# 3decomp/poissbox

Hardware: AMD Instinct MI355X
Metric: CG iter/s and DoF-updates/s at 512^3; achieved HBM GB/s vs peak (higher is better)
Workload: dtype f64

## Files before the change

### poissbox_amd/csrc/pb_cg_device.hpp

```cpp
#pragma once

#include <type_traits>
#include <utility>
#include "pb_device.hpp"

namespace pb {

__device__ __forceinline__ bool finite(double v) { return v == v && v - v == 0.0; }
__device__ __forceinline__ double norm_from_sq(double zz) { return sqrt(zz < 0.0 ? 0.0 : zz); }
template <class S>
__device__ __forceinline__ void ablate_keep_going(S& st) {
#ifdef PB_ABLATE_NO_EXITS
  if (st.reason != PB_KSP_DIVERGED_ITS) st.reason = 0, st.done = 0;
#endif
}

static constexpr int kFoldMaxParts = 1024;
static constexpr int kMaxSums = 5;
__device__ __forceinline__ void wave_reduce_parts(const double* __restrict__ parts, int nparts,
                                                  int width, double* S) {
  const int lane = threadIdx.x & 63;
#pragma unroll
  for (int s = 0; s < kMaxSums; ++s) {
    double v = 0.0;
// ... 165 lines not shown
    } else if (skip && i + 1 >= st.max_it) {
      st.beta = zr;
      st.mu = mu;
      st.delta = S[4];
      st.it = i + 1;
      st.reason = PB_KSP_CONVERGED_ITS;
      st.done = 1;
    } else {
      st.beta = zr;
      st.mu = mu;
      st.delta = S[4];
      st.it = i + 1;
      if (!finite(zr)) {
        st.reason = PB_KSP_DIVERGED_NANORINF;
        st.done = 1;
      } else if (st.it >= st.max_it) {
        st.reason = PB_KSP_DIVERGED_ITS;
        st.done = 1;
      } else if (zr == 0.0) {
        st.its = st.it + 1;
        st.reason = PB_KSP_CONVERGED_ATOL;
        st.done = 1;
      } else if (zr * st.betaold < 0.0) {
        st.its = st.it + 1;
        st.reason = PB_KSP_DIVERGED_INDEFINITE_PC;
        st.done = 1;
      }
    }
  }
  ablate_keep_going(st);
  if (h_done) h_done[host_iter + 1] = st.done;
}

__device__ __forceinline__ void cg_sr_top(CgState& st) {
  if (st.done) return;
  const double dpi = st.it == 0 ? st.delta
                                : st.delta - st.beta * st.beta * st.dpi / (st.betaold * st.betaold);
  cg_stage1(st, dpi, false);
  if (!st.done) cg_pend(st);
}


__device__ __forceinline__ void cg_copy(CgState& d, const CgState& s) {
  d.beta = s.beta, d.betaold = s.betaold, d.dpi = s.dpi, d.dpiold = s.dpiold;
  d.alpha = s.alpha, d.alpha_prev = s.alpha_prev, d.mu = s.mu, d.dp = s.dp, d.ttol = s.ttol;
  d.rnorm0 = s.rnorm0, d.pa[0] = s.pa[0], d.pa[1] = s.pa[1], d.pa[2] = s.pa[2];
  d.rtol = s.rtol, d.atol = s.atol, d.dtol = s.dtol, d.dinv = s.dinv, d.ntot = s.ntot;
  d.it = s.it, d.its = s.its, d.max_it = s.max_it, d.nhist = s.nhist, d.pend_iter = s.pend_iter;
  d.pend_count = s.pend_count, d.nlog = s.nlog;
  d.reason = s.reason, d.done = s.done, d.pc = s.pc, d.nullspace = s.nullspace;
  d.defer_x = s.defer_x;
  d.bbp = s.bbp;
  d.delta = s.delta, d.sr = s.sr, d.norm = s.norm;
}
static_assert(sizeof(CgState) == 248, "cg_copy lists every CgState field");

__device__ __forceinline__ void fold_prologue(const Fold& f, CgState& st) {
  double S[kMaxSums];
  cg_copy(st, *f.in);
  if (f.stage != 4) wave_reduce_parts(f.parts, f.nparts, f.width, S);
  const bool lead = blockIdx.x == 0 && threadIdx.x == 0;
  if (f.stage == 1) {
    cg_stage1(st, S[0]);
  } else if (f.stage == 2) {
    cg_stage2(st, S, lead ? f.hist : nullptr, lead ? f.h_done : nullptr, f.host_iter);
  } else {
// ... 58 lines not shown
```

### poissbox_amd/csrc/pb_cg_passes.hip

```cpp
#include "pb_star7.hpp"

namespace pb {

struct CombineLoad {
  static constexpr int NR = 2;
  static constexpr bool GHOST_RAW = false;
  const double* __restrict__ r;
  const double* __restrict__ p;
  const CgState* st;
  double dinv, shift, bb;
  int after1 = 0;
  __device__ __forceinline__ void prepare() { prepare_from(*st); }
  template <class S>
  __device__ __forceinline__ void prepare_from(const S& s) {
    dinv = s.dinv;
    shift = -s.mu;
    bb = after1 ? s.bbp : (s.it == 0 ? 0.0 : s.beta / s.betaold);
  }
  __device__ __forceinline__ const double* src(int a) const { return a == 0 ? r : p; }
  __device__ __forceinline__ double f(double rv, double pv) const {
    double z = dinv * rv;
    z = z + shift;
    return z + bb * pv;
  }
// ... 499 lines not shown
                          double* p_new, const StencilPlanes& gp, const Fold& fold, int mode,
                          int part_off, int* nblocks, bool store) {
  ScopedTimer tm(g->ctx,
                 timer_name(mode, "cg_pass_a", "cg_pass_a_interior", "cg_pass_a_boundary"));
  const CombineLoad ld{r, p_old, nullptr, 0.0, 0.0, 0.0};
  Launch lc = Launch{nullptr, mode}.sums(part_off, nblocks);
  lc.fold = fold;
  if (!store) return launch_any(g, s, ld, gp, PassAT<false>{p_new}, lc);
  return launch_any(g, s, ld, gp, PassA{p_new}, lc);
}

int cg_reduce_allreduce(pb_ctx* ctx, int nparts, int width, bool b_region) {
  return cg_reduce_allreduce(ctx, ctx->d_partials + (b_region ? fold_parts_b_off(ctx) * 4 : 0),
                             nparts, width);
}

int cg_reduce_allreduce(pb_ctx* ctx, const double* parts, int nparts, int width) {
  hipLaunchKernelGGL(cg_finalize_kernel, dim3(1), dim3(256), 0, ctx->stream, parts, nparts, width,
                     ctx->d_scalars, 1, 0, (CgState*)nullptr, (double*)nullptr, (int*)nullptr,
                     (int64_t)0, RrParts{});
  PB_HIP(hipGetLastError());
  return allreduce_device(ctx, ctx->d_scalars, width);
}

int cg_stage2_from_sums(pb_ctx* ctx, int width, CgState* st, double* hist, int* h_done,
                        int64_t host_iter) {
  hipLaunchKernelGGL(cg_finalize_kernel, dim3(1), dim3(256), 0, ctx->stream,
                     (const double*)nullptr, 0, width, ctx->d_scalars, 2, 2, st, hist, h_done,
                     host_iter, RrParts{});
  PB_HIP(hipGetLastError());
  return PB_OK;
}

int cg_finalize_init(pb_ctx* ctx, int nparts, CgState* st, double* hist, int* h_done,
                     const RrParts& rr) {
  return cg_reduce_update(ctx, 0, nparts, 4, st, hist, h_done, -1, nullptr, rr);
}

int cg_finalize_pass_a(pb_ctx* ctx, int nparts, CgState* st) {
  return cg_reduce_update(ctx, 1, nparts, 1, st, nullptr, nullptr, 0);
}

int cg_finalize_stage2(pb_ctx* ctx, int nparts, CgState* st, double* hist, int* h_done,
                       int64_t host_iter, const RrParts& rr) {
  return cg_reduce_update(ctx, 2, nparts, 4, st, hist, h_done, host_iter, nullptr, rr);
}

template <int XU, bool PST>
static int pass_b_one(pb_grid* g, const Star& s, const double* p, const double* const* p_prev,
                      double* x, double* r, const StencilPlanes& gp, CgState* st, const Fold& f,
                      const PStore& ps, int* nparts, int part_off = 0) {
  const int* skip = f.stage ? nullptr : &st->done;
  const int off = f.stage ? (int)fold_parts_b_off(g->ctx) : part_off;
  Launch lc = Launch{skip}.sums(off, nparts);
  lc.rev = 1;
  lc.fold = f;
  PassB<XU, PST> ep{x, r, p_prev[0], XU == 3 ? p_prev[1] : nullptr, XU == 3 ? p_prev[2] : nullptr,
                    st, 0.0, 0.0, 0.0, 0.0, 0.0, 0.0};
  if constexpr (PST) {
    ep.r_out = ps.r_out;
    ep.p_out = const_cast<double*>(p);
    CombineLoad ld{ps.zsrc, p_prev[0], st, 0.0, 0.0, 0.0};
    ld.after1 = 1;
    return launch_any(g, s, ld, gp, ep, lc);
  } else {
    return launch_any(g, s, PlainLoad{p}, gp, ep, lc);
// ... 151 lines not shown
```

### poissbox_amd/csrc/pb_fft.hip

```cpp
#include <algorithm>
#include <cmath>
#include <vector>

#include "pb_internal.hpp"
#include "pb_device.hpp"

#pragma clang fp contract(fast)

namespace pb {

namespace {

struct DhtPass {
  const double* in;
  double* out;
  int64_t li, lo, es;
  int64_t lo_out;
  int esh_in, esh_out;
  int64_t ebs_in, ebs_out, es_out;
  int ninner, nouter, ntiles_inner;
  const double* w;
  const double* tab;
  int nx, ny, j0;
  double scale, thr;
  int remap;
  const double* sr;
  double* parts;
  const CgState* st;
  int nparts_out;
  int ncu;
  const double* ru_in;
  const double* ru_w;
  double* ru_out;
  const double* ru_p;
  double* ru_x;
  int ru_first;
  const CgState* ru_st;
  const double* in_alt = nullptr;
  double* out_alt = nullptr;
  int alt_blk = -1;
  int ablate;
};
#ifndef PB_FFT_ABLATE_TRAFFIC
#define PB_FFT_ABLATE_TRAFFIC 0
#endif

struct cplx {
  double re, im;
};
typedef double dv2 __attribute__((ext_vector_type(2)));
__device__ __forceinline__ cplx cmul(cplx a, cplx b) {
  return {a.re * b.re - a.im * b.im, a.re * b.im + a.im * b.re};
}
__device__ __forceinline__ cplx cadd(cplx a, cplx b) { return {a.re + b.re, a.im + b.im}; }
__device__ __forceinline__ cplx csub(cplx a, cplx b) { return {a.re - b.re, a.im - b.im}; }
__device__ __forceinline__ cplx cmi(cplx a) { return {a.im, -a.re}; }
__device__ __forceinline__ cplx cpi(cplx a) { return {-a.im, a.re}; }
__device__ __forceinline__ cplx cscale(cplx a, double s) { return {a.re * s, a.im * s}; }

__host__ __device__ constexpr int natural_radix_at(int n, int p) {
  int rest = n;
  for (int q = 0; q <= p; ++q) {
// ... 359 lines not shown
    const int f = fv + q * NS;
    if (NP % NS != 0 && f >= NP) {
      l = TL;
      e = 0;
    } else if (WAVE) {
      l = l0 + f / (N / 2);
      e = (f % (N / 2)) * 2;
    } else {
      l = (f % (TL / 2)) * 2;
      e = f / (TL / 2);
    }
  };
  constexpr bool PF = LAYOUT == 1 && N <= 512;
  dv2 pre[PF ? NR : 1];
  auto load_pair = [&](int64_t base, int nl, int q) -> dv2 {
    int l, e;
    coord(q, l, e);
    const bool ok = l < nl;
    const int lc = ok ? l : 0, ec = ok ? e : 0;
    if (PB_FFT_ABLATE_TRAFFIC) return dv2{0.0, 0.0};
    const double* src = p.in;
    if (LAYOUT == 0 && p.esh_in && (ec >> p.esh_in) == p.alt_blk) src = p.in_alt;
    return __builtin_nontemporal_load((const dv2*)(src + base + lc * p.li + eoff_in(ec)));
  };
  auto fetch = [&](int t) {
    int64_t outer, base;
    int inner0, nl;
    tile_of(t, outer, inner0, nl, base);
    if constexpr (PF) {
#pragma unroll
      for (int q = 0; q < NR; ++q) pre[q] = load_pair(base, nl, q);
    }
  };
  double acc[4] = {0.0, 0.0, 0.0, 0.0};
  const double mu = SUMS ? p.st->mu : 0.0;
  const int G = PF ? (int)gridDim.x : ntiles;
  int t = PF ? (int)blockIdx.x : xcd_block(p.remap);
  if (PF && t < ntiles) fetch(t);
  for (; t < ntiles; t += G) {
    int64_t outer, base;
    int inner0, nl;
    tile_of(t, outer, inner0, nl, base);

    if (WAVE)
      wave_sync_lds();
    else
      __syncthreads();
    auto put = [&](int l, int e, dv2 v) {
      if (LAYOUT == 0) {
        lds[l * LP + lpad(e)] = v.x;
        lds[(l + 1) * LP + lpad(e)] = v.y;
      } else {
        lds[l * LP + lpad(e)] = v.x;
        lds[l * LP + lpad(e + 1)] = v.y;
      }
    };
    if constexpr (PF) {
#pragma unroll
      for (int q = 0; q < NR; ++q) {
        int l, e;
        coord(q, l, e);
        if (l < nl) put(l, e, pre[q]);
      }
    } else {
      constexpr int QB = N <= 512 ? (NR < 8 ? NR : 8) : 4;
#pragma unroll
      for (int q0 = 0; q0 < NR; q0 += QB) {
        dv2 v[QB];
// ... 22 lines not shown
        fft_passes<N, 0, 1>(A, B, tw, lane);
        scale_combine2<N>(A, B, p, lane, outer, inner0 + l0);
        fft_passes<N, 0, 1>(A, B, tw, lane);
      } else {
        dht2<N>(A, B, tw, lane);
      }
    }
    if (WAVE)
      wave_sync_lds();
    else
      __syncthreads();
#pragma unroll
    for (int q = 0; q < NR; ++q) {
      int l, e;
      coord(q, l, e);
      if (l < nl) {
        dv2 v;
        if (LAYOUT == 0) {
          v.x = lds[l * LP + lpad(e)];
          v.y = lds[(l + 1) * LP + lpad(e)];
          if (MODE == 1) v.y = -v.y;
        } else {
          v.x = lds[l * LP + lpad(e)];
          v.y = lds[l * LP + lpad(e + 1)];
        }
        const int64_t a = base + outer * (p.lo_out - p.lo) + l * p.li + eoff_out(e);
        if (PB_FFT_ABLATE_TRAFFIC) {
          if (v.x == 12345.678) p.out[a] = v.y;
          continue;
        }
        double* dst = p.out;
        if (LAYOUT == 0 && p.esh_out && (e >> p.esh_out) == p.alt_blk) dst = p.out_alt;
        __builtin_nontemporal_store(v, (dv2*)(dst + a));
        if constexpr (SUMS) {
          const dv2 rv = __builtin_nontemporal_load((const dv2*)(p.sr + a));
          const double t0 = v.x - mu, t1 = v.y - mu;
          acc[0] += t0;
          acc[1] += t0 * t0;
          acc[2] += t0 * rv.x;
          acc[3] += rv.x;
          acc[0] += t1;
          acc[1] += t1 * t1;
          acc[2] += t1 * rv.y;
          acc[3] += rv.y;
        }
      }
    }
  }
  if constexpr (SUMS) {
    __syncthreads();
#pragma unroll
    for (int q = 0; q < 4; ++q) {
      double v = acc[q];
#pragma unroll
      for (int off = 32; off >= 1; off >>= 1) v += __shfl_xor(v, off, 64);
      if (lane == 0) lds[wave * 4 + q] = v;
    }
    __syncthreads();
    if (threadIdx.x < 4) {
      double v = lds[threadIdx.x];
      for (int w = 1; w < NT / 64; ++w) v += lds[w * 4 + threadIdx.x];
      p.parts[(int64_t)blockIdx.x * 4 + threadIdx.x] = v;
    }
  }
}

template <int N, bool SUMS, bool RUPD>
__global__ __launch_bounds__(512, N <= 512 ? 4 : 2) void dht_reg_x_kernel(DhtPass p,
                                                                          const int* skip) {
  static_assert(!(SUMS && RUPD), "sums on the last pass, the r update on the first");
  using RP = RegPlan<N>;
  static_assert(RP::OK, "register-edge plan");
  constexpr int R = RP::R, NB = RP::NB, T = RP::T;
  constexpr int TL = 16, LP = (lpad_max(N) + 1) | 1;
  constexpr bool TWL = N <= 512;
  if (skip && *skip) {
    if (RUPD && p.ru_first) {
      const int tile = blockIdx.x;
      const int64_t outer = tile / p.ntiles_inner;
      const int inner0 = (tile % p.ntiles_inner) * TL;
      const int nl = min(TL, p.ninner - inner0);
      for (int i = threadIdx.x; i < nl * N; i += 512)
        p.ru_x[outer * p.lo + (int64_t)(inner0 + i / N) * p.li + i % N] = 0.0;
    }
    return;
  }
  extern __shared__ __attribute__((aligned(16))) double lds[];
  const int lane = threadIdx.x & 63, wave = threadIdx.x >> 6;
  const double* tw = p.w;
  if constexpr (TWL) {
    double* twl = lds + TL * LP;
    for (int i = threadIdx.x; i < N; i += 512) {
      const dv2 c = *(const dv2*)(p.w + 2 * i);
      twl[2 * i] = c.x;
      twl[2 * i + 1] = c.y;
// ... 122 lines not shown
      PB_HIP(hipFuncSetAttribute((const void*)k, hipFuncAttributeMaxDynamicSharedMemorySize,
                                 (int)LDS));
    attr = true;
  }
  if (p.ru_st) {
    if (p.parts) return set_error(PB_ERR_STATE, "fft pc: r update and sums on one pass");
    kern = kern_r;
  }
  if (ntiles > INT32_MAX) return set_error(PB_ERR_UNSUPPORTED, "fft pc: too many tiles");
  int64_t nblocks = ntiles;
  if (p.parts) {
    static int occ = 0;
    if (!occ) {
      PB_HIP(hipOccupancyMaxActiveBlocksPerMultiprocessor(&occ, kern_s, 512, LDS));
      if (occ < 1) occ = 1;
    }
    nblocks = std::min<int64_t>(ntiles, (int64_t)occ * ctx->num_cus);
    if (nblocks * 4 > ctx->partials_cap)
      return set_error(PB_ERR_UNSUPPORTED, "fft pc: %lld blocks exceed the partials capacity",
                       (long long)nblocks);
    p.nparts_out = (int)nblocks;
    kern = kern_s;
  }
  hipLaunchKernelGGL(kern, dim3((unsigned)nblocks), dim3(512), LDS, ctx->stream, p, skip);
  PB_HIP(hipGetLastError());
  return PB_OK;
}

template <int N, int TL, int LAYOUT, int MODE>
int launch_dht_k(pb_ctx* ctx, DhtPass& p, const int* skip) {
  using T = DhtTile<N, TL>;
  p.ntiles_inner = (p.ninner + T::TL - 1) / T::TL;
  const int64_t ntiles = (int64_t)p.ntiles_inner * p.nouter;
  constexpr bool SUMS = LAYOUT == 1 && MODE == 0;
  auto kern = dht_lines_kernel<N, TL, LAYOUT, MODE, false>;
  auto kern_s = dht_lines_kernel<N, TL, LAYOUT, MODE, SUMS>;
  static int occ = 0;
  if (!occ) {
    PB_HIP(hipFuncSetAttribute((const void*)kern, hipFuncAttributeMaxDynamicSharedMemorySize,
                               (int)T::LDS));
    PB_HIP(hipFuncSetAttribute((const void*)kern_s, hipFuncAttributeMaxDynamicSharedMemorySize,
                               (int)T::LDS));
    PB_HIP(hipOccupancyMaxActiveBlocksPerMultiprocessor(&occ, kern_s, T::NT, T::LDS));
    if (occ < 1) occ = 1;
  }
  int64_t nblocks = (int64_t)occ * ctx->num_cus;
  const bool persist = N <= 512 && LAYOUT == 1;
  if (!persist || nblocks > ntiles) nblocks = ntiles;
  if (p.parts) {
    if (!SUMS) return set_error(PB_ERR_STATE, "fft pc: residual sums on the X pass only");
    if (nblocks * 4 > ctx->partials_cap)
      return set_error(PB_ERR_UNSUPPORTED, "fft pc: %lld blocks exceed the partials capacity",
                       (long long)nblocks);
    p.nparts_out = (int)nblocks;
    kern = kern_s;
  }
  hipLaunchKernelGGL(kern, dim3((unsigned)nblocks), dim3(T::NT), T::LDS, ctx->stream, p, skip);
  PB_HIP(hipGetLastError());
  return PB_OK;
}

template <int N, int LAYOUT, int MODE>
int launch_dht_n(pb_ctx* ctx, DhtPass& p, const int* skip) {
  if (p.ninner % 2)
    return set_error(PB_ERR_UNSUPPORTED, "fft pc: %d lines (even counts only)", p.ninner);
  if constexpr (RegPlan<N>::OK && LAYOUT == 1) return launch_dht_reg_x<N>(ctx, p, skip);
  if (p.ru_st) return set_error(PB_ERR_STATE, "fft pc: r update on the register-edge X pass only");
  return launch_dht_k<N, tile_lines<N>(), LAYOUT, MODE>(ctx, p, skip);
}

#define PB_FFT_LENGTHS(X) \
  X(32) X(64) X(128) X(256) X(512) X(1024) X(48) X(96) X(192) X(384) X(768) X(40) X(80) \
  X(160) X(320) X(640)

template <int LAYOUT, int MODE>
int launch_dht(pb_ctx* ctx, int64_t n, DhtPass& p, const int* skip) {
  switch (n) {
#define PB_FFT_CASE(L)                                                 \
  case L:                                                              \
    static_assert(plan_complete(L), "length without a Stockham plan"); \
    return launch_dht_n<L, LAYOUT, MODE>(ctx, p, skip);
    PB_FFT_LENGTHS(PB_FFT_CASE)
#undef PB_FFT_CASE
  }
// ... 99 lines not shown
  }
  pb_ctx* ctx = g->ctx;
  PB_HIP(hipMemcpyAsync(f->dev, host.data(), host.size() * sizeof(double), hipMemcpyHostToDevice,
                        ctx->stream));
  PB_SYNC(ctx, "fft pc tables");
  f->tw[0] = f->dev;
  f->tw[1] = f->dev + 2 * g->n[0];
  f->tw[2] = f->dev + 2 * (g->n[0] + g->n[1]);
  f->tab = f->dev + 2 * nsum;
  if (grid_split(g)) {
    const int64_t len = yslab_len(g) + yslab_aux_len(g);
    if (hipMalloc(&f->ybuf, (size_t)len * sizeof(double)) != hipSuccess) {
      (void)hipFree(f->dev);
      delete f;
      return set_error(PB_ERR_ALLOC, "fft pc y-slab buffer: out of device memory");
    }
  } else if (const int64_t pad = tune("fft_zpad", 32);
             pad > 0 && g->plane >= tune("fft_zpad_min_plane", 512 * 512)) {
    f->zplane = g->plane + pad;
    if (hipMalloc(&f->zbuf, (size_t)(f->zplane * g->nzl) * sizeof(double)) != hipSuccess) {
      (void)hipGetLastError();
      f->zbuf = nullptr;
      f->zplane = 0;
    }
  }
  *out = f;
  return PB_OK;
}

static int dht_axis(pb_ctx* ctx, const FftPc* f, const int64_t b[3], int axis, const double* in,
                    double* out, const int* skip, int j0 = 0, const double* sr = nullptr,
                    const CgState* st = nullptr, int* np = nullptr,
                    const RUpdate* ru = nullptr, int64_t pl_in = 0, int64_t pl_out = 0,
                    const YSlabPlan* blk = nullptr, int blk_dir = 0) {
  static const char* names[3] = {"pc_fft_x", "pc_fft_y", "pc_fft_z"};
  ScopedTimer tm(ctx, names[axis]);
  DhtPass p{};
  p.remap = 1;
  p.ablate = PB_ABLATE_FFT;
  p.ncu = ctx->num_cus;
  p.in = in;
  p.out = out;
  p.w = f->tw[axis];
  const int64_t nx = b[0], ny = b[1], nz = b[2];
  if (axis == 0) {
    p.li = nx;
    p.lo = nx * ny;
    p.lo_out = p.lo;
    p.es = 1;
    p.ninner = (int)ny;
    p.nouter = (int)nz;
    if (np) {
      p.sr = sr;
      p.st = st;
      p.parts = ctx->d_partials;
    }
    if (ru) {
      p.ru_in = ru->r_in;
      p.ru_w = ru->w;
      p.ru_out = ru->r_out;
      p.ru_p = ru->p;
      p.ru_x = ru->x;
      p.ru_first = ru->first;
      p.ru_st = ru->st;
    }
    PB_TRY((launch_dht<1, 0>(ctx, nx, p, skip)));
    if (np) *np = p.nparts_out;
// ... 9 lines not shown
    if (blk) {
      const int64_t nyl = blk->nyl[0];
      int sh = 0;
      while (((int64_t)1 << sh) < nyl) ++sh;
      if (blk_dir == 1) {
        p.lo_out = nyl * nx;
        p.esh_out = sh;
        p.ebs_out = nz * nyl * nx;
      } else {
        p.lo = nyl * nx;
        p.esh_in = sh;
        p.ebs_in = nz * nyl * nx;
      }
      if (blk->self_direct) {
        p.alt_blk = blk->me;
        p.out_alt = blk->alt_out;
        p.in_alt = blk->alt_out;
      }
    }
    return launch_dht<0, 0>(ctx, ny, p, skip);
  }
  p.li = 1;
  p.lo = nx;
  p.lo_out = nx;
  p.es = pl_in ? pl_in : nx * ny;
  p.ninner = (int)nx;
  p.nouter = (int)ny;
  p.tab = f->tab;
  p.nx = (int)f->g->n[0];
  p.ny = (int)f->g->n[1];
  p.j0 = j0;
  p.scale = 1.0 / ((double)f->g->n[0] * (double)f->g->n[1] * (double)f->g->n[2]);
  p.thr = f->thr;
  return launch_dht<0, 1>(ctx, nz, p, skip);
}

bool fftpc_fuses_r_update(const FftPc* f) {
  return (f->g->n[0] == 512 || f->g->n[0] == 1024) && f->g->n[1] % 2 == 0;
}

int fftpc_apply(FftPc* f, const double* r, double* z, const int* skip, const CgState* sums_st,
                int* nparts, const RUpdate* ru) {
  if (nparts) *nparts = 0;
  pb_grid* g = f->g;
  pb_ctx* ctx = g->ctx;
  if (ru && !fftpc_fuses_r_update(f))
    return set_error(PB_ERR_STATE, "fft pc: r update needs the register-edge X pass");
  ScopedTimer tm(ctx, "pc_fft");
  const int64_t b[3] = {g->n[0], g->n[1], g->nzl};
  PB_TRY(dht_axis(ctx, f, b, 0, r, z, skip, 0, nullptr, nullptr, nullptr, ru));
  if (f->zbuf) {
    PB_TRY(dht_axis(ctx, f, b, 1, z, f->zbuf, skip, 0, nullptr, nullptr, nullptr, nullptr, 0,
                    f->zplane));
    PB_TRY(dht_axis(ctx, f, b, 2, f->zbuf, f->zbuf, skip, 0, nullptr, nullptr, nullptr, nullptr,
                    f->zplane, f->zplane));
    PB_TRY(dht_axis(ctx, f, b, 1, f->zbuf, z, skip, 0, nullptr, nullptr, nullptr, nullptr,
                    f->zplane, 0));
  } else if (!grid_split(g)) {
    PB_TRY(dht_axis(ctx, f, b, 1, z, z, skip));
    PB_TRY(dht_axis(ctx, f, b, 2, z, z, skip));
    PB_TRY(dht_axis(ctx, f, b, 1, z, z, skip));
  } else {
    YSlabPlan yp;
    double* fy = f->ybuf;
    PB_TRY(yslab_begin(g, fy + yslab_len(g), &yp));
    const int64_t by[3] = {g->n[0], yp.ny_me, g->n[2]};
    if (yslab_blocked(yp)) {
      yp.alt_out = fy + yp.self_shift;
      PB_TRY(dht_axis(ctx, f, b, 1, z, yp.stage, skip, 0, nullptr, nullptr, nullptr, nullptr, 0,
                      0, &yp, 1));
      PB_TRY(alltoallv_device(ctx, yp.stage, yp.zc.data(), fy, yp.yc.data(), yp.self_direct));
      PB_TRY(dht_axis(ctx, f, by, 2, fy, fy, skip, (int)yp.j0[ctx->rank]));
      PB_TRY(alltoallv_device(ctx, fy, yp.yc.data(), yp.stage, yp.zc.data(), yp.self_direct));
      PB_TRY(dht_axis(ctx, f, b, 1, yp.stage, z, skip, 0, nullptr, nullptr, nullptr, nullptr, 0,
                      0, &yp, 2));
    } else {
      PB_TRY(dht_axis(ctx, f, b, 1, z, z, skip));
      PB_TRY(yslab_to(g, yp, z, fy));
      PB_TRY(dht_axis(ctx, f, by, 2, fy, fy, skip, (int)yp.j0[ctx->rank]));
      PB_TRY(yslab_from(g, yp, fy, z));
      PB_TRY(dht_axis(ctx, f, b, 1, z, z, skip));
    }
  }
  if (sums_st && nparts) return dht_axis(ctx, f, b, 0, z, z, skip, 0, r, sums_st, nparts);
  return dht_axis(ctx, f, b, 0, z, z, skip);
}

void fftpc_destroy(FftPc* f) {
  if (!f) return;
  (void)wait_stream(f->g->ctx, f->g->ctx->stream, "fftpc_destroy");
  if (f->dev) (void)hipFree(f->dev);
  if (f->ybuf) (void)hipFree(f->ybuf);
  if (f->zbuf) (void)hipFree(f->zbuf);
  delete f;
}

}
```

### poissbox_amd/csrc/pb_internal.hpp

```cpp
#pragma once

#include <hip/hip_runtime.h>
#include <rccl/rccl.h>
#include <rocprofiler-sdk-roctx/roctx.h>

#include <cstdint>
#include <cstdio>
#include <deque>
#include <map>
#include <string>
#include <functional>
#include <vector>

#include "poissbox_gpu.h"

namespace pb {

int set_error(int code, const char* fmt, ...);

#define PB_HIP(call)                                                                    \
  do {                                                                                  \
    hipError_t e_ = (call);                                                             \
    if (e_ != hipSuccess)                                                               \
      return ::pb::set_error(PB_ERR_HIP, "%s:%d %s: %s", __FILE__, __LINE__, #call,     \
// ... 446 lines not shown
                       const double* q, const double* b, double* y_out, double* r_out,
                       const StencilPlanes& gp, const CgState* st, double scale, bool sums,
                       int* nparts, int part_off = 0);
int launch_cheb_x(pb_grid* g, const double* y, const double* ym1, const double* q, double* y_out,
                  const CgState* st, double scale);
int launch_pre_scale_sum(pb_grid* g, const double* src, double* dst, double dinv, int* nparts);
int launch_pre_shift(pb_grid* g, double* x, double ntot);

struct Mg;
int mg_create(pb_grid* g, const double deltas[3], int pc_type, int levels_req, int coarse_its,
              double omega, Mg** out);
int mg_apply(Mg* mg, const double* r, double* z, const int* skip = nullptr,
             const CgState* sums_st = nullptr, int* nparts = nullptr);
int mg_levels(const Mg* mg);
struct MgSmoother {
  int ksp = 0, pc = 0, nu = 1;
  double rich_scale = 1.0, emin = 0.0, emax = 0.0;
};
int mg_set_smoother(Mg* mg, const MgSmoother& sm);
void mg_destroy(Mg* mg);
int mg_plan_levels(const int64_t n[3], int nranks, int levels_req);

struct FftPc;
int fftpc_create(pb_grid* g, const double deltas[3], int compact, FftPc** out);
struct RUpdate {
  const double* r_in;
  const double* w;
  double* r_out;
  const double* p;
  double* x;
  int first;
  const CgState* st;
};
int fftpc_apply(FftPc* f, const double* r, double* z, const int* skip = nullptr,
                const CgState* sums_st = nullptr, int* nparts = nullptr,
                const RUpdate* ru = nullptr);
bool fftpc_fuses_r_update(const FftPc* f);
void fftpc_destroy(FftPc* f);

int ctx_scratch(pb_ctx* ctx, size_t n, double** out);

int reduce_partials(pb_ctx* ctx, const double* parts, int nparts, int width, double* out);

}
```

### poissbox_amd/csrc/pb_ksp.hpp

```cpp
#pragma once
#include <vector>

#include "pb_internal.hpp"

namespace pb {
struct FgState;
struct PcgState;
}

struct pb_ksp {
  pb_op* A = nullptr;
  pb_op* P = nullptr;
  pb_ksp_opts opts;
  int norm_type = PB_KSP_NORM_DEFAULT;
  int norm() const {
    if (norm_type != PB_KSP_NORM_DEFAULT) return norm_type;
    if (opts.ksp_type == PB_KSP_FGMRES) return PB_KSP_NORM_UNPRECONDITIONED;
    return opts.ksp_type == PB_KSP_PREONLY ? PB_KSP_NORM_NONE : PB_KSP_NORM_PRECONDITIONED;
  }
  bool norm_none() const { return norm() == PB_KSP_NORM_NONE; }
  bool norm_unp() const { return norm() == PB_KSP_NORM_UNPRECONDITIONED; }
  int64_t solve_iters() const {
    return norm_none() ? opts.max_it : opts.max_it + 2 * (int64_t)opts.check_every;
  }
// ... 66 lines not shown
  pb_vec* x = nullptr;
  int64_t host_iter = 0;
  bool stopped = false;
  bool begun = false;
  int defer_x = 4;
  int pslots() const { return defer_x == 4 ? 4 : 2; }
  struct Sr {
    bool on = false;
    int nparts = 0;
  };
  Sr sr;
  struct Fischer {
    int maxl = 0, curl = 0;
    std::vector<double*> xt, bt;
    double* guess = nullptr;
    double* d_coef = nullptr;
  };
  Fischer* fg = nullptr;
};

#pragma GCC visibility push(hidden)
namespace pb {

inline bool fused_kind(int kind) { return kind == PB_OP_STAR7; }

int op_apply_raw(pb_op* op, const double* x, double* y);
struct OpApplySkip {
  pb_ctx* ctx;
  OpApplySkip(pb_ctx* c, const int* flag) : ctx(c) { ctx->op_skip = flag; }
  ~OpApplySkip() { ctx->op_skip = nullptr; }
};

int ensure_done_cap(pb_ksp* k, int64_t need);
int pc_apply_dev(pb_ksp* k, const double* r, double* z, const int* skip, int* np);

int check_cheb_pair(double emin, double emax, const char* what);
int check_cheb_opts(const pb_ksp_chebyshev_opts* o);
int check_mg_opts(const pb_pc_mg_opts* o);
int check_guess_opts(int model, int maxl);
int check_ref_norm_opts(const pb_ksp_opts* o);
int check_richardson_scale(double scale);
void mg_levels_bounds(const pb_pc_mg_opts* o, double* emin, double* emax);

int rich_begin(pb_ksp* k, const pb_vec* b, pb_vec* x);
int enqueue_rich_iteration(pb_ksp* k);
int rich_copy_back(pb_ksp* k, int64_t its);
int solve_preonly(pb_ksp* k, const pb_vec* b, pb_vec* x, pb_ksp_result* res);

int fgmres_create(pb_ksp* k);
int fgmres_begin(pb_ksp* k, const pb_vec* b, pb_vec* x);
int enqueue_fgmres_iteration(pb_ksp* k);
int fgmres_finish(pb_ksp* k);
void fgmres_destroy(pb_ksp* k);
int check_fgmres_opts(const pb_ksp_fgmres_opts* o);

constexpr int kFgMaxRestart = 64;
constexpr int kFgLd = kFgMaxRestart + 1;
struct FgState {
  double hh[kFgLd * kFgMaxRestart];
  double cs[kFgMaxRestart], sn[kFgMaxRestart];
  double g[kFgLd];
  double y[kFgMaxRestart];
  double dots[kFgLd], dots2[kFgLd];
  double nrm2;
  double wsum;
  double shift;
  double bsq;
// ... 61 lines not shown
```

### poissbox_amd/csrc/pb_runtime.cpp

```cpp
#include <time.h>

#include <algorithm>
#include <atomic>
#include <chrono>
#include <cstdarg>
#include <cstdlib>
#include <cstring>
#include <condition_variable>
#include <memory>
#include <mutex>
#include <string>
#include <thread>
#include <unordered_map>

#include "pb_internal.hpp"

namespace pb {

hipError_t field_alloc(void** p, size_t bytes) { return hipMalloc(p, bytes); }

void field_free(void* p) {
  if (p) (void)hipFree(p);
}

namespace {
const char* const kTuneNames[] = {
    "a2a_copy_self", "cg_defer_x", "engine_kc_skew", "cg_fold", "cg_fuse", "cg_sr_fused", "cheb_fused", "comm_mark_every",
    "comm_stall_test_ms", "compact_lines", "fft_rupd", "fgmres_fused", "pipecg_fused", "fft_zpad", "fft_zpad_min_plane",
    "force_comm", "ksp_lazy0", "mg_agglomerate", "mg_engine_min_plane", "mg_poly_fused", "mg_restrict_z_min_cols",
    "mg_split_fused", "mg_sweep2", "mg_tail_max", "mg_u4_split", "pcr_lines", "rich_fused", "sor_omega_any", "sr_ddiff",
    "stencil_kc", "stencil_kc_skew", "stencil_nt", "stencil_tall", "stencil_wgcu", "x_dot_cu"};
constexpr int kNumTune = (int)(sizeof(kTuneNames) / sizeof(kTuneNames[0]));
std::atomic<int> g_tune_val[kNumTune];
std::atomic<int> g_tune_set[kNumTune];
std::atomic<int> g_tune_nset{0};
int tune_index(const char* name) {
  for (int i = 0; i < kNumTune; ++i)
    if (strcmp(kTuneNames[i], name) == 0) return i;
  return -1;
}
}

int tune(const char* name, int dflt) {
  if (g_tune_nset.load(std::memory_order_acquire) == 0) return dflt;
  const int i = tune_index(name);
  if (i < 0 || !g_tune_set[i].load(std::memory_order_acquire)) return dflt;
  return g_tune_val[i].load(std::memory_order_relaxed);
}

bool tune_is_set(const char* name) {
  const int i = tune_index(name);
  return i >= 0 && g_tune_set[i].load(std::memory_order_acquire) != 0;
}

static thread_local char g_err[1024] = "";

int set_error(int code, const char* fmt, ...) {
  va_list ap;
  va_start(ap, fmt);
  vsnprintf(g_err, sizeof(g_err), fmt, ap);
  va_end(ap);
// ... 1027 lines not shown
```

### poissbox_amd/csrc/pb_solver.cpp

```cpp
#include <cmath>
#include <cstdio>
#include <cstring>
#include <string>
#include <vector>

#include "pb_ksp.hpp"

using namespace pb;

static int sr_pass_s(pb_ksp* k, const double* r, const CgState* st, int* nparts, int64_t n);
static const double* sr_region(const pb_ctx* ctx, int64_t n);
static int cg_begin(pb_ksp* k, const pb_vec* b, pb_vec* x, CgState& st);

int pb::ensure_done_cap(pb_ksp* k, int64_t need) {
  if (need <= k->done_cap) return PB_OK;
  int64_t cap = need < 1024 ? 1024 : need * 2;
  int* h = nullptr;
  PB_HIP(hipHostMalloc(&h, (size_t)cap * sizeof(int), hipHostMallocMapped));
  memset(h, 0, (size_t)cap * sizeof(int));
  if (k->h_done) {
    PB_TRY(wait_stream(k->A->grid->ctx, k->A->grid->ctx->stream, "KSP flag buffer"));
    memcpy(h, k->h_done, (size_t)k->done_cap * sizeof(int));
    (void)hipHostFree(k->h_done);
  }
  k->h_done = h;
  PB_HIP(hipHostGetDevicePointer((void**)&k->h_done_dev, h, 0));
  k->done_cap = cap;
  return PB_OK;
}

int pb::pc_apply_dev(pb_ksp* k, const double* r, double* z, const int* skip, int* np) {
  *np = 0;
  if (k->fft) return fftpc_apply(k->fft, r, z, skip, k->d_st, np);
  return mg_apply(k->mg, r, z, skip, k->d_st, np);
}

extern "C" {

int pb_ksp_create(pb_op* A, pb_op* P, const pb_ksp_opts* opts, pb_ksp** out) {
  PB_CHECK_ARG(A && out, "bad ksp args");
  if (!P) P = A;
  PB_CHECK_ARG(A->grid == P->grid, "A and P on different grids");
  pb_ksp* k = new pb_ksp();
  k->A = A;
  k->P = P;
  auto fail = [k](int rc) {
    const std::string msg = pb_last_error();
    pb_ksp_destroy(k);
    return set_error(rc, "%s", msg.c_str());
  };
  if (opts) k->opts = *opts;
  else pb_ksp_opts_default(&k->opts);
  if (k->opts.check_every < 1) k->opts.check_every = 8;
  if (check_ref_norm_opts(&k->opts) != PB_OK) return fail(PB_ERR_ARG);
  const int kt = k->opts.ksp_type;
  if (kt != PB_KSP_CG && kt != PB_KSP_PREONLY && kt != PB_KSP_RICHARDSON &&
      kt != PB_KSP_CHEBYSHEV && kt != PB_KSP_FGMRES && kt != PB_KSP_PIPECG)
    return fail(set_error(PB_ERR_UNSUPPORTED, "unknown ksp_type %d", kt));
  pb_ksp_chebyshev_opts_default(&k->ch.opts);
  pb_pc_mg_opts_default(&k->mgopts);
  if (const int rc = fgmres_create(k)) return fail(rc);
  if (const int rc = pipecg_create(k)) return fail(rc);
  if (check_richardson_scale(k->opts.richardson_scale) != PB_OK) return fail(PB_ERR_ARG);
  if (kt == PB_KSP_PREONLY &&
      (k->opts.initial_guess_nonzero || k->opts.guess_type != PB_GUESS_NONE))
    return fail(set_error(PB_ERR_ARG,
// ... 212 lines not shown
    if (k->norm_unp()) PB_TRY(launch_cg_rr(g, r0, &rr));
    PB_TRY(pc_apply_dev(k, r0, k->z, nullptr, &np));
    if (np == 0) PB_TRY(launch_cg_pc_sums(g, k->z, r0, k->d_st, &np));
    PB_TRY(cg_finalize_init(ctx, np, k->d_st, k->d_hist, k->h_done_dev, rr));
  } else {
    PB_TRY(launch_cg_init(g, b->d, x->d, k->r, k->pb[0], k->d_st, st.dinv, k->d_hist,
                          k->h_done_dev));
    if (k->sr.on) {
      int np = 0;
      PB_TRY(sr_pass_s(k, k->r, k->d_st, &np, 0));
      PB_TRY(cg_sr_finalize(ctx, sr_region(ctx, 0), np, k->d_st, k->d_hist, k->h_done_dev, -1,
                            true));
    }
  }
  return PB_OK;
}

static int enqueue_generic_iteration(pb_ksp* k) {
  pb_grid* g = k->A->grid;
  pb_ctx* ctx = g->ctx;
  double* p = k->pb[0];
  int np = 0;
  PB_TRY(launch_cg_generic_p(g, k->r, p, k->d_st));
  {
    OpApplySkip guard(ctx, &k->d_st->done);
    PB_TRY(op_apply_raw(k->A, p, k->w));
  }
  PB_TRY(launch_cg_generic_dot(g, p, k->w, k->d_st, &np));
  PB_TRY(cg_finalize_pass_a(ctx, np, k->d_st));
  PB_TRY(launch_cg_generic_xr(g, p, k->w, k->x->d, k->r, k->d_st, &np));
  return cg_finalize_stage2(ctx, np, k->d_st, k->d_hist, k->h_done_dev, k->host_iter);
}

static int enqueue_pc_iteration(pb_ksp* k) {
  pb_grid* g = k->A->grid;
  pb_ctx* ctx = g->ctx;
  double* p = k->pb[0];
  int np = 0;
  const int first = k->lazy0 && k->host_iter == 0;
  if (k->A->kind == PB_OP_COMPACT && (compact_cg_fusable(g) || compact_cg_fusable_split(g))) {
    CgFuse cf;
    cf.z = k->z;
    cf.p_old = p;
    cf.p_out = p;
    cf.st = k->d_st;
    cf.first = first;
    cf.dot_p = p;
    {
      OpApplySkip guard(ctx, &k->d_st->done);
      struct Set {
        pb_ctx* c;
        ~Set() { c->cg_fuse = nullptr; }
      } set{ctx};
      ctx->cg_fuse = &cf;
      PB_TRY(op_apply_raw(k->A, p, k->w));
    }
    np = cf.nparts;
    if (!cf.fused_z) {
      PB_TRY(launch_cg_generic_p(g, k->z, p, k->d_st, first));
      OpApplySkip guard(ctx, &k->d_st->done);
      PB_TRY(op_apply_raw(k->A, p, k->w));
    }
    if (!cf.fused_z || !cf.fused_dot) PB_TRY(launch_cg_generic_dot(g, p, k->w, k->d_st, &np));
  } else {
    PB_TRY(launch_cg_generic_p(g, k->z, p, k->d_st, first));
    {
      OpApplySkip guard(ctx, &k->d_st->done);
      PB_TRY(op_apply_raw(k->A, p, k->w));
    }
    PB_TRY(launch_cg_generic_dot(g, p, k->w, k->d_st, &np));
  }
  PB_TRY(cg_finalize_pass_a(ctx, np, k->d_st));
  const double* r_in = first ? k->b->d : k->r;
  const int rupd = tune("fft_rupd", 1);
  RrParts rr;
  const bool unp = k->norm_unp();
  if (k->fft && rupd && fftpc_fuses_r_update(k->fft) && !unp) {
    const RUpdate ru{r_in, k->w, k->r, p, k->x->d, first, k->d_st};
    np = 0;
    PB_TRY(fftpc_apply(k->fft, k->r, k->z, &k->d_st->done, k->d_st, &np, &ru));
  } else {
    PB_TRY(launch_cg_pc_xr(g, p, k->w, k->x->d, r_in, k->r, k->d_st, first, unp ? &rr : nullptr));
    PB_TRY(pc_apply_dev(k, k->r, k->z, &k->d_st->done, &np));
  }
  if (np == 0) PB_TRY(launch_cg_pc_sums(g, k->z, k->r, k->d_st, &np));
  return cg_finalize_stage2(ctx, np, k->d_st, k->d_hist, k->h_done_dev, k->host_iter, rr);
}

static int64_t sr_region_off(const pb_ctx* ctx, int64_t n) {
  return (n & 1) * (ctx->partials_cap / 10);
}
static const double* sr_region(const pb_ctx* ctx, int64_t n) {
  return ctx->d_partials + sr_region_off(ctx, n) * 5;
}

static int sr_pass_s(pb_ksp* k, const double* r, const CgState* st, int* nparts, int64_t n) {
  pb_grid* g = k->A->grid;
  pb_ctx* ctx = g->ctx;
  const Star s = star_of(k->A);
  StencilPlanes gp;
  const int off = (int)sr_region_off(ctx, n);
  const int end = off + (int)(ctx->partials_cap / 10);
  if (!ctx->split) {
    gp = wrap_planes();
    return launch_cg_sr_pass_s(g, s, r, gp, st, PLANES_ALL, off, end, nparts);
  }
  gp.ghost_lo = g->ghost_lo;
  gp.ghost_hi = g->ghost_hi;
  const double* hi = r + (g->nzl - 1) * g->plane;
  if (g->nzl < 3) {
    PB_TRY(halo_exchange(g, r, hi));
    return launch_cg_sr_pass_s(g, s, r, gp, st, PLANES_ALL, off, end, nparts);
  }
  int nb1 = 0, nb2 = 0;
  ScopedTimer tm(ctx, "cg_sr_s");
  PB_TRY(halo_begin(g, r, hi));
// ... 171 lines not shown
  }
  if (!ctx->split) {
    gp = wrap_planes();
    PB_TRY(launch_cg_pass_a(g, s, zsrc, p_old, p_new, gp, k->d_st, PLANES_ALL, 0, &nparts,
                            store_a));
  } else if (g->nzl < 3) {
    PB_TRY(launch_cg_boundary(g, zsrc, p_old, k->d_st));
    PB_TRY(halo_exchange(g, g->bnd_lo, g->bnd_hi));
    gp.ghost_lo = g->ghost_lo;
    gp.ghost_hi = g->ghost_hi;
    PB_TRY(launch_cg_pass_a(g, s, zsrc, p_old, p_new, gp, k->d_st, PLANES_ALL, 0, &nparts,
                            store_a));
  } else {
    PB_TRY(launch_cg_boundary(g, zsrc, p_old, k->d_st));
    gp.ghost_lo = g->ghost_lo;
    gp.ghost_hi = g->ghost_hi;
    int nb1 = 0, nb2 = 0;
    ScopedTimer tm(ctx, "cg_pass_a");
    PB_TRY(halo_begin(g, g->bnd_lo, g->bnd_hi));
    PB_TRY(launch_cg_pass_a(g, s, zsrc, p_old, p_new, gp, k->d_st, PLANES_INTERIOR, 0, &nb1,
                            store_a));
    PB_TRY(halo_end(g));
    PB_TRY(launch_cg_pass_a(g, s, zsrc, p_old, p_new, gp, k->d_st, PLANES_BOUNDARY, nb1, &nb2,
                            store_a));
    nparts = nb1 + nb2;
  }
  PB_TRY(cg_finalize_pass_a(ctx, nparts, k->d_st));
  RrParts rr;
  PB_TRY(launch_cg_pass_b(g, s, p_new, p_prev, k->x->d, r, gp, k->d_st, k->d_hist,
                          k->h_done_dev, i, k->defer_x, !k->stored_z(), ps,
                          k->stored_z() && k->norm_unp() ? &rr : nullptr));
  if (k->stored_z()) {
    int np = 0;
    PB_TRY(pc_apply_dev(k, r, k->z, &k->d_st->done, &np));
    if (np == 0) PB_TRY(launch_cg_pc_sums(g, k->z, r, k->d_st, &np));
    PB_TRY(cg_finalize_stage2(ctx, np, k->d_st, k->d_hist, k->h_done_dev, i, rr));
  }
  return PB_OK;
}

int pb_ksp_iterate(pb_ksp* k, int64_t iters) {
  PB_CHECK_ARG(k, "ksp is NULL");
  PB_TRY(preonly_split_form(k));
  if (!k->begun) return set_error(PB_ERR_STATE, "pb_ksp_iterate before pb_ksp_begin");
  pb_ctx* ctx = k->A->grid->ctx;
  const int C = k->opts.check_every;
  const int R = 4 * C;
  if ((int)k->ring.size() < R) {
    for (int i = (int)k->ring.size(); i < R; ++i) {
      hipEvent_t e;
      PB_HIP(hipEventCreateWithFlags(&e, hipEventDisableTiming));
      k->ring.push_back(e);
    }
  }
  PB_TRY(ensure_done_cap(k, k->host_iter + iters + 2));
  const bool fold = C >= 2 && !k->rich() && !k->fgmres() && !k->pipecg() &&
                    fused_kind(k->A->kind) &&
                    !k->stored_z() && tune("cg_fold", 1) != 0;
  const bool none = k->norm_none();
  int64_t n = 0;
  for (; n < iters && !k->stopped; ++n) {
    if (k->rich()) PB_TRY(enqueue_rich_iteration(k));
    else if (k->fgmres()) PB_TRY(enqueue_fgmres_iteration(k));
    else if (k->pipecg()) PB_TRY(enqueue_pipecg_iteration(k));
    else if (k->sr.on) PB_TRY(enqueue_sr_iteration(k, fold, n));
    else PB_TRY(enqueue_iteration(k, fold, fold && n > 0));
    const int64_t hi = k->host_iter++;
// ... 235 lines not shown
```

Measured before the change: 107.0 billion.

## Compute preconditioned residual norm in spectral space for early CG exit

Accumulates z-norm sums (sum of squares and the zero mode) during the FFT preconditioner's Z pass. A small kernel then evaluates the convergence test using Parseval before the inverse Y transform, marking the solve done early so the remaining passes are skipped on the converged iteration. This adds one tiny reduction kernel per iteration, plus an allreduce in split mode, in exchange for skipping the tail of the final iteration.

```diff
diff --git a/poissbox_amd/csrc/pb_cg_device.hpp b/poissbox_amd/csrc/pb_cg_device.hpp
--- a/poissbox_amd/csrc/pb_cg_device.hpp
+++ b/poissbox_amd/csrc/pb_cg_device.hpp
@@ -221,6 +221,35 @@
   if (h_done) h_done[host_iter + 1] = st.done;
 }
 
+__device__ __forceinline__ void cg_stage2_early(CgState& st, double sz, double szz, double* hist,
+                                                int* h_done, int64_t host_iter) {
+  if (st.done || st.norm != PB_KSP_NORM_PRECONDITIONED) return;
+  const double N = st.ntot, mu = st.mu;
+  const int64_t i = st.it;
+  const double s0 = sz - N * mu;
+  const double s1 = szz - 2.0 * mu * sz + N * mu * mu;
+  double zz = s1;
+  if (st.nullspace) {
+    const double delta = s0 / N;
+    zz = s1 - N * delta * delta;
+  }
+  const double dp = norm_from_sq(zz);
+  if (!finite(dp) || !(dp <= st.ttol)) return;
+#ifdef PB_ABLATE_NO_EXITS
+  return;
+#endif
+  if (!st.sr) cg_pend(st);
+  st.dp = dp;
+  st.its = i + 1;
+  if (i + 1 < st.nhist) {
+    if (hist) hist[i + 1] = dp;
+    st.nlog = i + 2;
+  }
+  st.reason = dp < st.atol ? PB_KSP_CONVERGED_ATOL : PB_KSP_CONVERGED_RTOL;
+  st.done = 1;
+  if (h_done) h_done[host_iter + 1] = 1;
+}
+
 __device__ __forceinline__ void cg_sr_top(CgState& st) {
   if (st.done) return;
   const double dpi = st.it == 0 ? st.delta
diff --git a/poissbox_amd/csrc/pb_cg_passes.hip b/poissbox_amd/csrc/pb_cg_passes.hip
--- a/poissbox_amd/csrc/pb_cg_passes.hip
+++ b/poissbox_amd/csrc/pb_cg_passes.hip
@@ -555,6 +555,53 @@
   return PB_OK;
 }
 
+__global__ __launch_bounds__(256) void cg_early_norm_kernel(const double* __restrict__ parts,
+                                                            int nparts, double* sums, int mode,
+                                                            double xy, CgState* st, double* hist,
+                                                            int* h_done, int64_t host_iter) {
+  if (st->done) return;
+  if (mode & 1) {
+    __shared__ double red[256][2];
+    double v0 = 0.0, v1 = 0.0;
+    for (int b = threadIdx.x; b < nparts; b += 256) {
+      v0 += parts[(int64_t)b * 2];
+      v1 += parts[(int64_t)b * 2 + 1];
+    }
+    red[threadIdx.x][0] = v0;
+    red[threadIdx.x][1] = v1;
+    __syncthreads();
+    for (int off = 128; off >= 1; off >>= 1) {
+      if ((int)threadIdx.x < off) {
+        red[threadIdx.x][0] += red[threadIdx.x + off][0];
+        red[threadIdx.x][1] += red[threadIdx.x + off][1];
+      }
+      __syncthreads();
+    }
+    if (threadIdx.x == 0) sums[0] = red[0][0], sums[1] = red[0][1];
+  }
+  if (!(mode & 2) || threadIdx.x != 0) return;
+  cg_stage2_early(*st, xy * sums[0], xy * sums[1], hist, h_done, host_iter);
+}
+
+int cg_early_norm(pb_ctx* ctx, const double* parts, int nparts, double xy, const EarlyNorm& e) {
+  ScopedTimer tm(ctx, "cg_early_norm");
+  double* sums = ctx->d_scalars;
+  if (!ctx->split) {
+    hipLaunchKernelGGL(cg_early_norm_kernel, dim3(1), dim3(256), 0, ctx->stream, parts, nparts,
+                       sums, 3, xy, e.st, e.hist, e.h_done, e.host_iter);
+    PB_HIP(hipGetLastError());
+    return PB_OK;
+  }
+  hipLaunchKernelGGL(cg_early_norm_kernel, dim3(1), dim3(256), 0, ctx->stream, parts, nparts,
+                     sums, 1, xy, e.st, e.hist, e.h_done, e.host_iter);
+  PB_HIP(hipGetLastError());
+  PB_TRY(allreduce_device(ctx, sums, 2));
+  hipLaunchKernelGGL(cg_early_norm_kernel, dim3(1), dim3(256), 0, ctx->stream, parts, nparts,
+                     sums, 2, xy, e.st, e.hist, e.h_done, e.host_iter);
+  PB_HIP(hipGetLastError());
+  return PB_OK;
+}
+
 int cg_finalize_init(pb_ctx* ctx, int nparts, CgState* st, double* hist, int* h_done,
                      const RrParts& rr) {
   return cg_reduce_update(ctx, 0, nparts, 4, st, hist, h_done, -1, nullptr, rr);
diff --git a/poissbox_amd/csrc/pb_fft.hip b/poissbox_amd/csrc/pb_fft.hip
--- a/poissbox_amd/csrc/pb_fft.hip
+++ b/poissbox_amd/csrc/pb_fft.hip
@@ -28,6 +28,7 @@
   double* parts;
   const CgState* st;
   int nparts_out;
+  int zsums;
   int ncu;
   const double* ru_in;
   const double* ru_w;
@@ -453,8 +454,10 @@
       for (int q = 0; q < NR; ++q) pre[q] = load_pair(base, nl, q);
     }
   };
+  constexpr bool XS = SUMS && MODE == 0, ZS = SUMS && MODE == 1;
+  static_assert(!ZS || LAYOUT == 0, "spectral sums on the strided Z pass");
   double acc[4] = {0.0, 0.0, 0.0, 0.0};
-  const double mu = SUMS ? p.st->mu : 0.0;
+  const double mu = XS ? p.st->mu : 0.0;
   const int G = PF ? (int)gridDim.x : ntiles;
   int t = PF ? (int)blockIdx.x : xcd_block(p.remap);
   if (PF && t < ntiles) fetch(t);
@@ -543,7 +546,13 @@
         double* dst = p.out;
         if (LAYOUT == 0 && p.esh_out && (e >> p.esh_out) == p.alt_blk) dst = p.out_alt;
         __builtin_nontemporal_store(v, (dv2*)(dst + a));
-        if constexpr (SUMS) {
+        if constexpr (ZS) {
+          const bool line0 = inner0 + l == 0 && p.j0 + (int)outer == 0;
+          acc[0] += line0 ? v.x : 0.0;
+          acc[1] += v.x * v.x;
+          acc[1] += v.y * v.y;
+        }
+        if constexpr (XS) {
           const dv2 rv = __builtin_nontemporal_load((const dv2*)(p.sr + a));
           const double t0 = v.x - mu, t1 = v.y - mu;
           acc[0] += t0;
@@ -559,19 +568,20 @@
     }
   }
   if constexpr (SUMS) {
+    constexpr int W = ZS ? 2 : 4;
     __syncthreads();
 #pragma unroll
-    for (int q = 0; q < 4; ++q) {
+    for (int q = 0; q < W; ++q) {
       double v = acc[q];
 #pragma unroll
       for (int off = 32; off >= 1; off >>= 1) v += __shfl_xor(v, off, 64);
-      if (lane == 0) lds[wave * 4 + q] = v;
+      if (lane == 0) lds[wave * W + q] = v;
     }
     __syncthreads();
-    if (threadIdx.x < 4) {
+    if (threadIdx.x < W) {
       double v = lds[threadIdx.x];
-      for (int w = 1; w < NT / 64; ++w) v += lds[w * 4 + threadIdx.x];
-      p.parts[(int64_t)blockIdx.x * 4 + threadIdx.x] = v;
+      for (int w = 1; w < NT / 64; ++w) v += lds[w * W + threadIdx.x];
+      p.parts[(int64_t)blockIdx.x * W + threadIdx.x] = v;
     }
   }
 }
@@ -760,7 +770,8 @@
   using T = DhtTile<N, TL>;
   p.ntiles_inner = (p.ninner + T::TL - 1) / T::TL;
   const int64_t ntiles = (int64_t)p.ntiles_inner * p.nouter;
-  constexpr bool SUMS = LAYOUT == 1 && MODE == 0;
+  constexpr bool SUMS = (LAYOUT == 1 && MODE == 0) || (LAYOUT == 0 && MODE == 1);
+  constexpr int SW = MODE == 1 ? 2 : 4;
   auto kern = dht_lines_kernel<N, TL, LAYOUT, MODE, false>;
   auto kern_s = dht_lines_kernel<N, TL, LAYOUT, MODE, SUMS>;
   static int occ = 0;
@@ -776,8 +787,9 @@
   const bool persist = N <= 512 && LAYOUT == 1;
   if (!persist || nblocks > ntiles) nblocks = ntiles;
   if (p.parts) {
-    if (!SUMS) return set_error(PB_ERR_STATE, "fft pc: residual sums on the X pass only");
-    if (nblocks * 4 > ctx->partials_cap)
+    if (!SUMS || (MODE == 1) != (p.zsums != 0))
+      return set_error(PB_ERR_STATE, "fft pc: residual sums on the X pass, spectral on the Z pass");
+    if (nblocks * SW > ctx->partials_cap / (MODE == 1 ? 2 : 1))
       return set_error(PB_ERR_UNSUPPORTED, "fft pc: %lld blocks exceed the partials capacity",
                        (long long)nblocks);
     p.nparts_out = (int)nblocks;
@@ -943,7 +955,7 @@
                     double* out, const int* skip, int j0 = 0, const double* sr = nullptr,
                     const CgState* st = nullptr, int* np = nullptr,
                     const RUpdate* ru = nullptr, int64_t pl_in = 0, int64_t pl_out = 0,
-                    const YSlabPlan* blk = nullptr, int blk_dir = 0) {
+                    const YSlabPlan* blk = nullptr, int blk_dir = 0, int* znp = nullptr) {
   static const char* names[3] = {"pc_fft_x", "pc_fft_y", "pc_fft_z"};
   ScopedTimer tm(ctx, names[axis]);
   DhtPass p{};
@@ -1019,7 +1031,13 @@
   p.j0 = j0;
   p.scale = 1.0 / ((double)f->g->n[0] * (double)f->g->n[1] * (double)f->g->n[2]);
   p.thr = f->thr;
-  return launch_dht<0, 1>(ctx, nz, p, skip);
+  if (znp) {
+    p.parts = early_parts(ctx);
+    p.zsums = 1;
+  }
+  PB_TRY((launch_dht<0, 1>(ctx, nz, p, skip)));
+  if (znp) *znp = p.nparts_out;
+  return PB_OK;
 }
 
 bool fftpc_fuses_r_update(const FftPc* f) {
@@ -1027,7 +1045,7 @@
 }
 
 int fftpc_apply(FftPc* f, const double* r, double* z, const int* skip, const CgState* sums_st,
-                int* nparts, const RUpdate* ru) {
+                int* nparts, const RUpdate* ru, const EarlyNorm* early) {
   if (nparts) *nparts = 0;
   pb_grid* g = f->g;
   pb_ctx* ctx = g->ctx;
@@ -1035,17 +1053,26 @@
     return set_error(PB_ERR_STATE, "fft pc: r update needs the register-edge X pass");
   ScopedTimer tm(ctx, "pc_fft");
   const int64_t b[3] = {g->n[0], g->n[1], g->nzl};
+  int znp_ = 0;
+  int* znp = early ? &znp_ : nullptr;
+  auto early_stage = [&]() {
+    if (!early) return (int)PB_OK;
+    return cg_early_norm(ctx, early_parts(ctx), znp_, (double)g->n[0] * (double)g->n[1], *early);
+  };
   PB_TRY(dht_axis(ctx, f, b, 0, r, z, skip, 0, nullptr, nullptr, nullptr, ru));
   if (f->zbuf) {
     PB_TRY(dht_axis(ctx, f, b, 1, z, f->zbuf, skip, 0, nullptr, nullptr, nullptr, nullptr, 0,
                     f->zplane));
     PB_TRY(dht_axis(ctx, f, b, 2, f->zbuf, f->zbuf, skip, 0, nullptr, nullptr, nullptr, nullptr,
-                    f->zplane, f->zplane));
+                    f->zplane, f->zplane, nullptr, 0, znp));
+    PB_TRY(early_stage());
     PB_TRY(dht_axis(ctx, f, b, 1, f->zbuf, z, skip, 0, nullptr, nullptr, nullptr, nullptr,
                     f->zplane, 0));
   } else if (!grid_split(g)) {
     PB_TRY(dht_axis(ctx, f, b, 1, z, z, skip));
-    PB_TRY(dht_axis(ctx, f, b, 2, z, z, skip));
+    PB_TRY(dht_axis(ctx, f, b, 2, z, z, skip, 0, nullptr, nullptr, nullptr, nullptr, 0, 0, nullptr,
+                    0, znp));
+    PB_TRY(early_stage());
     PB_TRY(dht_axis(ctx, f, b, 1, z, z, skip));
   } else {
     YSlabPlan yp;
@@ -1057,14 +1084,18 @@
       PB_TRY(dht_axis(ctx, f, b, 1, z, yp.stage, skip, 0, nullptr, nullptr, nullptr, nullptr, 0,
                       0, &yp, 1));
       PB_TRY(alltoallv_device(ctx, yp.stage, yp.zc.data(), fy, yp.yc.data(), yp.self_direct));
-      PB_TRY(dht_axis(ctx, f, by, 2, fy, fy, skip, (int)yp.j0[ctx->rank]));
+      PB_TRY(dht_axis(ctx, f, by, 2, fy, fy, skip, (int)yp.j0[ctx->rank], nullptr, nullptr,
+                      nullptr, nullptr, 0, 0, nullptr, 0, znp));
+      PB_TRY(early_stage());
       PB_TRY(alltoallv_device(ctx, fy, yp.yc.data(), yp.stage, yp.zc.data(), yp.self_direct));
       PB_TRY(dht_axis(ctx, f, b, 1, yp.stage, z, skip, 0, nullptr, nullptr, nullptr, nullptr, 0,
                       0, &yp, 2));
     } else {
       PB_TRY(dht_axis(ctx, f, b, 1, z, z, skip));
       PB_TRY(yslab_to(g, yp, z, fy));
-      PB_TRY(dht_axis(ctx, f, by, 2, fy, fy, skip, (int)yp.j0[ctx->rank]));
+      PB_TRY(dht_axis(ctx, f, by, 2, fy, fy, skip, (int)yp.j0[ctx->rank], nullptr, nullptr,
+                      nullptr, nullptr, 0, 0, nullptr, 0, znp));
+      PB_TRY(early_stage());
       PB_TRY(yslab_from(g, yp, fy, z));
       PB_TRY(dht_axis(ctx, f, b, 1, z, z, skip));
     }
diff --git a/poissbox_amd/csrc/pb_internal.hpp b/poissbox_amd/csrc/pb_internal.hpp
--- a/poissbox_amd/csrc/pb_internal.hpp
+++ b/poissbox_amd/csrc/pb_internal.hpp
@@ -502,9 +502,17 @@
   int first;
   const CgState* st;
 };
+struct EarlyNorm {
+  CgState* st;
+  double* hist;
+  int* h_done;
+  int64_t host_iter;
+};
+inline double* early_parts(const pb_ctx* ctx) { return rr_region(ctx); }
+int cg_early_norm(pb_ctx* ctx, const double* parts, int nparts, double xy, const EarlyNorm& e);
 int fftpc_apply(FftPc* f, const double* r, double* z, const int* skip = nullptr,
                 const CgState* sums_st = nullptr, int* nparts = nullptr,
-                const RUpdate* ru = nullptr);
+                const RUpdate* ru = nullptr, const EarlyNorm* early = nullptr);
 bool fftpc_fuses_r_update(const FftPc* f);
 void fftpc_destroy(FftPc* f);
 
diff --git a/poissbox_amd/csrc/pb_ksp.hpp b/poissbox_amd/csrc/pb_ksp.hpp
--- a/poissbox_amd/csrc/pb_ksp.hpp
+++ b/poissbox_amd/csrc/pb_ksp.hpp
@@ -122,7 +122,8 @@
 };
 
 int ensure_done_cap(pb_ksp* k, int64_t need);
-int pc_apply_dev(pb_ksp* k, const double* r, double* z, const int* skip, int* np);
+int pc_apply_dev(pb_ksp* k, const double* r, double* z, const int* skip, int* np,
+                 const EarlyNorm* early = nullptr);
 
 int check_cheb_pair(double emin, double emax, const char* what);
 int check_cheb_opts(const pb_ksp_chebyshev_opts* o);
diff --git a/poissbox_amd/csrc/pb_runtime.cpp b/poissbox_amd/csrc/pb_runtime.cpp
--- a/poissbox_amd/csrc/pb_runtime.cpp
+++ b/poissbox_amd/csrc/pb_runtime.cpp
@@ -26,7 +26,7 @@
 namespace {
 const char* const kTuneNames[] = {
     "a2a_copy_self", "cg_defer_x", "engine_kc_skew", "cg_fold", "cg_fuse", "cg_sr_fused", "cheb_fused", "comm_mark_every",
-    "comm_stall_test_ms", "compact_lines", "fft_rupd", "fgmres_fused", "pipecg_fused", "fft_zpad", "fft_zpad_min_plane",
+    "comm_stall_test_ms", "compact_lines", "fft_early_norm", "fft_rupd", "fgmres_fused", "pipecg_fused", "fft_zpad", "fft_zpad_min_plane",
     "force_comm", "ksp_lazy0", "mg_agglomerate", "mg_engine_min_plane", "mg_poly_fused", "mg_restrict_z_min_cols",
     "mg_split_fused", "mg_sweep2", "mg_tail_max", "mg_u4_split", "pcr_lines", "rich_fused", "sor_omega_any", "sr_ddiff",
     "stencil_kc", "stencil_kc_skew", "stencil_nt", "stencil_tall", "stencil_wgcu", "x_dot_cu"};
diff --git a/poissbox_amd/csrc/pb_solver.cpp b/poissbox_amd/csrc/pb_solver.cpp
--- a/poissbox_amd/csrc/pb_solver.cpp
+++ b/poissbox_amd/csrc/pb_solver.cpp
@@ -29,9 +29,10 @@
   return PB_OK;
 }
 
-int pb::pc_apply_dev(pb_ksp* k, const double* r, double* z, const int* skip, int* np) {
+int pb::pc_apply_dev(pb_ksp* k, const double* r, double* z, const int* skip, int* np,
+                     const EarlyNorm* early) {
   *np = 0;
-  if (k->fft) return fftpc_apply(k->fft, r, z, skip, k->d_st, np);
+  if (k->fft) return fftpc_apply(k->fft, r, z, skip, k->d_st, np, nullptr, early);
   return mg_apply(k->mg, r, z, skip, k->d_st, np);
 }
 
@@ -310,6 +311,12 @@
   return cg_finalize_stage2(ctx, np, k->d_st, k->d_hist, k->h_done_dev, k->host_iter);
 }
 
+static bool early_norm_on(const pb_ksp* k) {
+  if (!k->fft || k->norm() != PB_KSP_NORM_PRECONDITIONED) return false;
+  const int v = tune("fft_early_norm", 1);
+  return v >= 2 || (v == 1 && !k->A->grid->ctx->split);
+}
+
 static int enqueue_pc_iteration(pb_ksp* k) {
   pb_grid* g = k->A->grid;
   pb_ctx* ctx = g->ctx;
@@ -353,13 +360,15 @@
   const int rupd = tune("fft_rupd", 1);
   RrParts rr;
   const bool unp = k->norm_unp();
+  const EarlyNorm en{k->d_st, k->d_hist, k->h_done_dev, k->host_iter};
+  const EarlyNorm* early = early_norm_on(k) ? &en : nullptr;
   if (k->fft && rupd && fftpc_fuses_r_update(k->fft) && !unp) {
     const RUpdate ru{r_in, k->w, k->r, p, k->x->d, first, k->d_st};
     np = 0;
-    PB_TRY(fftpc_apply(k->fft, k->r, k->z, &k->d_st->done, k->d_st, &np, &ru));
+    PB_TRY(fftpc_apply(k->fft, k->r, k->z, &k->d_st->done, k->d_st, &np, &ru, early));
   } else {
     PB_TRY(launch_cg_pc_xr(g, p, k->w, k->x->d, r_in, k->r, k->d_st, first, unp ? &rr : nullptr));
-    PB_TRY(pc_apply_dev(k, k->r, k->z, &k->d_st->done, &np));
+    PB_TRY(pc_apply_dev(k, k->r, k->z, &k->d_st->done, &np, early));
   }
   if (np == 0) PB_TRY(launch_cg_pc_sums(g, k->z, k->r, k->d_st, &np));
   return cg_finalize_stage2(ctx, np, k->d_st, k->d_hist, k->h_done_dev, k->host_iter, rr);
@@ -597,7 +606,8 @@
                           k->stored_z() && k->norm_unp() ? &rr : nullptr));
   if (k->stored_z()) {
     int np = 0;
-    PB_TRY(pc_apply_dev(k, r, k->z, &k->d_st->done, &np));
+    const EarlyNorm en{k->d_st, k->d_hist, k->h_done_dev, i};
+    PB_TRY(pc_apply_dev(k, r, k->z, &k->d_st->done, &np, early_norm_on(k) ? &en : nullptr));
     if (np == 0) PB_TRY(launch_cg_pc_sums(g, k->z, r, k->d_st, &np));
     PB_TRY(cg_finalize_stage2(ctx, np, k->d_st, k->d_hist, k->h_done_dev, i, rr));
   }
```

After: 107.0 billion (median of 2 runs). About the same (+0.0%).
